# techmum21p/hybrid-rag-ColBERTv2

Hardware: AMD Instinct MI355X
Metric: queries/sec + p50 retrieval latency, 1M-chunk corpus, top-10 rerank (higher is better)
Workload: dtype fp32 (faithful: bf16 hi/lo split, fp32 accumulate)

## Files before the change

hybrid-rag-colbertv2_amd/_lib.py:

```python
from __future__ import annotations

import ctypes
import os
import re

PKG = os.path.dirname(os.path.abspath(__file__))
LIB_PATH = os.path.join(PKG, "libcolbert_mi355x.so")
HEADER = os.path.join(os.path.dirname(PKG), "include", "colbert_mi355x.h")

DTYPE_BF16 = 1
DTYPE_F32 = 2
DTYPE_MXFP8 = 3
SCORER_MAXSIM = 0
SCORER_REF_MEANPOOL_COSINE = 1
SCORERS = {"maxsim": SCORER_MAXSIM, "ref_meanpool_cosine": SCORER_REF_MEANPOOL_COSINE}
ERR_EINVAL, ERR_EUNSUPPORTED, ERR_EHIP, ERR_ESTATE = -1, -2, -3, -4
F32_SCORE, F32_SEARCH, F32_RERANK = 0, 1, 2
(OPT_FUSED_TOPK, OPT_DYNAMIC_TAIL, OPT_BAND_DOC_MAJOR, OPT_BAND_LOWER_BOUND, OPT_TOPK_BMAX, OPT_BAND_FUSED,
 OPT_RESCORE_SPLIT, OPT_BAND_REUSE, OPT_BAND_BLOCK_SKIP, OPT_RESCORE_GRID, OPT_DENSE_DOCS, OPT_P1_COLLECT_FUSED,
 OPT_FOLD_KEYS, OPT_FILTER_PATH, OPT_FILTER_BATCH_CHUNK_DOCS, OPT_FILTER_BAND) = (1, 2, 3, 4, 5, 6, 7, 8, 9, 10, 11, 12,
                                                                                 13, 14, 15, 16)
FILTER_AUTO, FILTER_SUBSET, FILTER_DENSE = 0, 1, 2
FILTER_BAND_AUTO, FILTER_BAND_ON, FILTER_BAND_OFF = 0, 1, 2

_p, _i32, _i64, _sz = ctypes.c_void_p, ctypes.c_int32, ctypes.c_int64, ctypes.c_size_t
_SIGS = {
    "cbv2_abi_version": (ctypes.c_int, []),
    "cbv2_last_error": (ctypes.c_char_p, []),
    "cbv2_build_stamp": (ctypes.c_char_p, []),
    "cbv2_index_create": (ctypes.c_int, [ctypes.c_int, _p, _i32, _i64, _i32, _i32, _p, _i64,
                                         ctypes.POINTER(ctypes.c_void_p)]),
    "cbv2_index_destroy": (ctypes.c_int, [_p]),
    "cbv2_hbm_alloc": (ctypes.c_int, [ctypes.c_int, ctypes.c_size_t, ctypes.POINTER(ctypes.c_void_p),
                                      ctypes.POINTER(ctypes.c_int32)]),
    "cbv2_hbm_free": (ctypes.c_int, [ctypes.c_int, _p]),
    "cbv2_index_time_scans": (ctypes.c_int, [_p, _i32]),
# ... 139 lines not shown
```

hybrid-rag-colbertv2_amd/csrc/colbert_mi355x.hip:

```cpp
#include <hip/hip_runtime.h>

#include <stdarg.h>
#include <stdint.h>

#include <algorithm>
#include <atomic>
#include <mutex>
#include <type_traits>
#include <vector>
#include <stdio.h>
#include <string.h>

#include "colbert_mi355x.h"

namespace {

constexpr int kDim = 128;
constexpr int kLd = 128;
constexpr int kLqMax = 32;
constexpr int kRowBytes = kDim * 2;
constexpr int kDocBytes = kLd * kRowBytes;
constexpr int kTopkMax = 1024;
constexpr int kSmallMax = 1024;
constexpr int kMergeMax = 8192;
// ... 3516 lines not shown
  }
  __syncthreads();
  if (wave == 0) {
    const float m0 = fmaxf(fmaxf(s_m[0][c16], s_m[1][c16]), fmaxf(s_m[2][c16], s_m[3][c16]));
    const float m1 = fmaxf(fmaxf(s_m[0][16 + c16], s_m[1][16 + c16]), fmaxf(s_m[2][16 + c16], s_m[3][16 + c16]));
    const float v = dpp_row_sum16((c16 < lq ? m0 : 0.0f) + (16 + c16 < lq ? m1 : 0.0f));
    if (lane == 0) {
      raw[(size_t)b * C + c] = v;
      if (raw_words.w != nullptr) raw_words.put((size_t)b * C + c, (int32_t)__float_as_uint(v), 0.0f);
    }
  }
}

constexpr float kBoundUp = 1.0f + 1.0f / 1024.0f;
constexpr float kAccSlack = 1.0f / 4096.0f;

__device__ __forceinline__ void split_row8(const float* __restrict__ src, uint16_t* __restrict__ hi,
                                           uint16_t* __restrict__ lo, int sub, float& xx, float& rr, float& hh) {
  const f32x4* s4 = reinterpret_cast<const f32x4*>(src + 8 * sub);
  const f32x4 v0 = s4[0], v1 = s4[1];
  float x[8] = {v0[0], v0[1], v0[2], v0[3], v1[0], v1[1], v1[2], v1[3]};
  uint16_t h[8], l[8];
  xx = rr = hh = 0.0f;
#pragma unroll
  for (int e = 0; e < 8; ++e) {
    const __bf16 bh = (__bf16)x[e];
    const float fh = (float)bh;
    const float r = x[e] - fh;
    const __bf16 bl = (__bf16)r;
    h[e] = __builtin_bit_cast(uint16_t, bh);
// ... 45 lines not shown
}

constexpr int kArriveSlotsK = 4;
constexpr int kArrPhase1K = 3;
constexpr int64_t kSplitZeroInts = 16384;
__global__ __launch_bounds__(512) void split_query_kernel(const float* __restrict__ Q, int lq,
                                                          uint16_t* __restrict__ qhi, uint16_t* __restrict__ qlo,
                                                          float E, float M, float* __restrict__ beta,
                                                          int32_t* __restrict__ count = nullptr,
                                                          uint32_t* __restrict__ lbu = nullptr,
                                                          int32_t* __restrict__ done = nullptr, int count0 = 0,
                                                          int32_t* __restrict__ arrive = nullptr, int narrive = 0,
                                                          int* __restrict__ ctr = nullptr, int nctr = 0,
                                                          uint32_t ready_seq = 0, int nrows = 0,
                                                          uint32_t* __restrict__ zkeys = nullptr, int64_t nz = 0,
                                                          int32_t* __restrict__ ready_words = nullptr) {
  __shared__ float s_t[kLqMax];
  const int b = blockIdx.x, tid = threadIdx.x, r = tid >> 4, sub = tid & 15;
  if (nrows > 0 && b >= nrows) {
    const int64_t per = kSplitZeroInts, i0 = (int64_t)(b - nrows) * per;
    for (int64_t i = i0 + 4 * tid; i < i0 + per && i < nz; i += 4 * blockDim.x) {
      if (i + 3 < nz)
        *reinterpret_cast<uint4*>(zkeys + i) = make_uint4(0u, 0u, 0u, 0u);
      else
        for (int64_t e = i; e < nz; ++e) zkeys[e] = 0u;
    }
    return;
  }
  if (r < lq) {
    const size_t row = (size_t)b * lq + r;
    float xx, rr, hh;
    split_row8(Q + row * kDim, qhi + row * kDim, qlo + row * kDim, sub, xx, rr, hh);
    const float nq = sqrtf(xx) * kBoundUp, eq = sqrtf(rr) * kBoundUp;
    const float t = nq * E + eq * M + kAccSlack * (nq + eq) * M;
    if (sub == 0) s_t[r] = t;
  }
  __syncthreads();
  if (tid == 0) {
    float a[4];
#pragma unroll
    for (int g = 0; g < 4; ++g) {
      a[g] = 0.0f;
      for (int rr = g; rr < lq; rr += 4) a[g] += s_t[rr];
    }
    beta[b] = ((a[0] + a[1]) + (a[2] + a[3])) * kBoundUp;
    if (count != nullptr) count[b] = count0;
    if (lbu != nullptr) lbu[b] = 0xffffffffu;
    if (done != nullptr) done[b] = 0;
  }
  if (arrive != nullptr) {
    const int per = narrive / kArriveSlotsK;
    for (int i = tid; i < narrive; i += blockDim.x) {
      const int j = i / per, e = i - j * per;
      arrive[((size_t)j * nrows + b) * per + e] = 0;
    }
  }
  if (ctr != nullptr && b == 0)
    for (int i = tid; i < nctr; i += blockDim.x) ctr[i] = 0;
  if (ready_seq != 0 && ready_words != nullptr) {
    __syncthreads();
// ... 125 lines not shown
      if (16 * rt < dlb) {
        const f32x4 init = (dlb >= 16 * rt + 16) ? f32x4{} : row_mask_init16(16 * rt + 4 * g, dlb);
        tile16_x3(ah[t], al[t], qh, ql, init, m);
      }
    }
  }
  const float w0 = fold16_max(fold32_max(m[0])), w1 = fold16_max(fold32_max(m[1]));
  if (lane < 16) {
    s_m[wave][lane] = w0;
    s_m[wave][16 + lane] = w1;
  }
  __syncthreads();
  float v = 0.0f;
  if (wave == 0) {
    float m0 = s_m[0][c16], m1 = s_m[0][16 + c16];
#pragma unroll
    for (int w = 1; w < NW; ++w) {
      m0 = fmaxf(m0, s_m[w][c16]);
      m1 = fmaxf(m1, s_m[w][16 + c16]);
    }
    v = dpp_row_sum16((c16 < lq ? m0 : 0.0f) + (16 + c16 < lq ? m1 : 0.0f));
  }
  __syncthreads();
  return v;
}

struct RowSelect {
  int mode = 0;
  int32_t* arrive = nullptr;
  int k = 0;
// ... 83 lines not shown
    int r = 0;
    for (int j = 0; j < m; ++j) r += sel[j] > key ? 1 : 0;
    if (r < k) {
      os[r] = u2f((uint32_t)(key >> 32));
      oi[r] = (int32_t)(id_base + (int64_t)(~(uint32_t)key));
      if (mirror.w != nullptr) mirror.put(r, oi[r], os[r]);
    }
  }
  for (int j = m + tid; j < k; j += nth) {
    os[j] = neg_inf();
    oi[j] = -1;
    if (mirror.w != nullptr) mirror.put(j, -1, neg_inf());
  }
}

template <bool LONG = false, int NW = 4>
__global__ __launch_bounds__(NW * 64, 2) void rescore_split_kernel(
    const uint8_t* __restrict__ hi, const uint8_t* __restrict__ lo, const int32_t* __restrict__ doclens, int64_t n,
    int64_t id_base, const uint16_t* __restrict__ qhi, const uint16_t* __restrict__ qlo, int lq,
    const int32_t* __restrict__ cand, const int32_t* __restrict__ count, int64_t limit, int64_t ld_c,
    float* __restrict__ out, int64_t ld_out, const int32_t* __restrict__ only_neg, int ld,
    uint32_t* __restrict__ lb_min, int64_t c0, float* __restrict__ fb_T = nullptr, int32_t* __restrict__ fb_done = nullptr,
    int fb_k = 0, float* __restrict__ fb_s = nullptr, int32_t* __restrict__ fb_i = nullptr, RowSelect rs = RowSelect(),
    TaggedCand tc = TaggedCand()) {
  __shared__ float s_m[4][32];
  __shared__ uint64_t sel[kTopkMax];
  __shared__ uint32_t hist[2048];
  __shared__ uint32_t s_bin, s_above, s_bincount, s_cnt;
  __shared__ uint32_t misc[8];
  __shared__ int s_last;
  __shared__ int32_t s_cid;
  const int lane = threadIdx.x & 63;
  const int wave = __builtin_amdgcn_readfirstlane(threadIdx.x >> 6);
  const int b = blockIdx.y;
  if (rs.stamps != nullptr && threadIdx.x == 0 && blockIdx.x < kLabWgs)
    rs.stamps[16 + 2 * blockIdx.x] = __builtin_amdgcn_s_memrealtime();
  if (only_neg != nullptr && only_neg[b] >= 0) return;
  int64_t lim = limit;
  if (count != nullptr) {
// ... 16 lines not shown
      __threadfence();
      const int kk = (int)((int64_t)fb_k < n ? fb_k : n);
      topk_exact_row(row, n, kk, sel, hist, &s_bin, &s_above, &s_bincount, &s_cnt);
      sort_and_write(sel, kk, fb_k, id_base, fb_s + (size_t)b * fb_k, fb_i + (size_t)b * fb_k,
                     rs.ids_mirror.row(b, fb_k));
      if (rs.mode == kSelBand && threadIdx.x == 0) rs.status[b] = cb >= kWaitTimedOut ? -2 : -1;
      return;
    }
  }
  const bool idle = c0 + (int64_t)blockIdx.x >= lim;
  if (idle && rs.mode == kSelNone) return;
  if (!idle) {
    bf16x8 qh[2][4], ql[2][4];
    load_qfrag16(qhi, b, b + 1, lq, lane, qh);
    load_qfrag16(qlo, b, b + 1, lq, lane, ql);
    for (int64_t c = c0 + blockIdx.x; c < lim; c += gridDim.x) {
      int64_t id;
      if (tc.w != nullptr) {
        if (threadIdx.x == 0) {
          s_cid = wait_tagged(tc.w + (size_t)b * ld_c + c, tc);
          if (rs.mode != kSelNone)
            st_sc1(reinterpret_cast<uint32_t*>(const_cast<int32_t*>(cand)) + (size_t)b * ld_c + c, (uint32_t)s_cid);
        }
        __syncthreads();
        id = s_cid;
        __syncthreads();
      } else {
        id = cand ? (int64_t)cand[b * ld_c + c] : id_base + c;
      }
      const int64_t loc = id - id_base;
      float v = neg_inf();
      if (id >= 0 && loc >= 0 && loc < n)
        v = faithful_doc_split<LONG, NW>(hi, lo, loc, ld, doclens[loc], qh, ql, lane, wave, lq, s_m);
      if (threadIdx.x == 0) {
        if (rs.mode != kSelNone)
          st_sc1(out + (size_t)b * ld_out + c, v);
        else
          out[(size_t)b * ld_out + c] = v;
        if (rs.raw.w != nullptr) rs.raw.put((size_t)b * ld_c + c, (int32_t)__float_as_uint(v), 0.0f);
        if (lb_min != nullptr) atomicMin(lb_min + b, f2u(v));
      }
    }
  }
  if (rs.stamps != nullptr && threadIdx.x == 0 && blockIdx.x < kLabWgs)
    rs.stamps[17 + 2 * blockIdx.x] = __builtin_amdgcn_s_memrealtime();
  if (rs.mode == kSelNone) return;
  if (!row_last_arrival(rs.arrive + (size_t)b * kArriveInts, (int)gridDim.x, 8, &s_last)) return;
  lab_stamp(rs.stamps, 6);
// ... 331 lines not shown
      __syncthreads();
    }
    d = d_next;
  }
}

__device__ __forceinline__ float band_threshold(int b, const float* __restrict__ lb, const uint32_t* __restrict__ lbu,
                                                const float* __restrict__ topk_s, int k,
                                                const float* __restrict__ beta) {
  if (lbu != nullptr) return u2f(lbu[b]) - beta[b];
  if (lb != nullptr) return lb[b] - beta[b];
  return topk_s[(size_t)b * k + k - 1] - 2.0f * beta[b];
}

constexpr int kBandLds = 2048;
__global__ __launch_bounds__(256) void band_collect_kernel(const float* __restrict__ T, int64_t n,
                                                           const float* __restrict__ topk_s, int k,
                                                           const float* __restrict__ beta, int64_t id_base,
                                                           int cap, int32_t* __restrict__ cand,
                                                           int32_t* __restrict__ count,
                                                           const float* __restrict__ lb,
                                                           const uint32_t* __restrict__ lbu,
                                                           const int32_t* __restrict__ topk_i,
                                                           const uint32_t* __restrict__ bm,
                                                           uint64_t* __restrict__ stamps = nullptr) {
  __shared__ int32_t s_ids[kBandLds];
  __shared__ int s_n, s_base;
  const int b = blockIdx.y, lane = threadIdx.x & 63;
  if (stamps != nullptr && threadIdx.x == 0 && blockIdx.x < kLabWgs)
    stamps[16 + 2 * blockIdx.x] = __builtin_amdgcn_s_memrealtime();
  if (threadIdx.x == 0) s_n = 0;
  __syncthreads();
  const float thr = band_threshold(b, lb, lbu, topk_s, k, beta);
  const float* row = T + (size_t)b * n;
  int32_t* crow = cand + (size_t)b * cap;
  uint64_t kth = 0;
  if (topk_i != nullptr) {
    kth = rank_key(topk_s[(size_t)b * k + k - 1], (uint32_t)((int64_t)topk_i[(size_t)b * k + k - 1] - id_base));
    if (blockIdx.x == 0)
      for (int j = threadIdx.x; j < k; j += blockDim.x) crow[j] = topk_i[(size_t)b * k + j];
  }
  auto offer = [&](int64_t i, float v) {
    const bool take = i < n && v >= thr && (topk_i == nullptr || rank_key(v, (uint32_t)i) < kth);
    const uint64_t mask = __ballot(take);
    if (mask == 0) return;
    const int nh = __popcll(mask);
    int base = 0;
    if (lane == 0) base = atomicAdd(&s_n, nh);
    base = __shfl(base, 0);
    const int pos = base + __popcll(mask & ((1ull << lane) - 1ull));
    if (take) {
      if (pos < kBandLds) {
        s_ids[pos] = (int32_t)(id_base + i);
      } else {
        const int gp = atomicAdd(count + b, 1);
        if (gp < cap) crow[gp] = (int32_t)(id_base + i);
      }
    }
  };
  if (bm != nullptr) {
    const int64_t nb = (n + 63) >> 6;
    const uint32_t* krow = bm + (size_t)b * nb;
    const uint32_t uthr = f2u(thr);
    const int wave = threadIdx.x >> 6, nw = blockDim.x >> 6;
    const int c16 = lane & 15, r4 = lane >> 4;
    const bool vec = (n & 3) == 0 && (reinterpret_cast<uintptr_t>(T) & 15) == 0;
    for (int64_t g0 = (int64_t)blockIdx.x * 64; g0 < nb; g0 += (int64_t)gridDim.x * 64) {
      const int64_t kb = g0 + lane;
      const uint64_t qual = __ballot(kb < nb && krow[kb] >= uthr);
      uint64_t mine = 0;
      int q = 0;
      for (uint64_t m = qual; m != 0; m &= m - 1, ++q)
        if (q % nw == wave) mine |= m & (~m + 1);
      while (mine != 0) {
        int64_t i0[4];
#pragma unroll
        for (int s4 = 0; s4 < 4; ++s4) {
          int64_t blk = -1;
#pragma unroll
          for (int u = 0; u < 4; ++u) {
            const int64_t bu = mine != 0 ? g0 + (__ffsll((long long)mine) - 1) : -1;
            if (mine != 0) mine &= mine - 1;
            if (u == r4) blk = bu;
          }
          i0[s4] = blk >= 0 ? (blk << 6) + 4 * c16 : n;
        }
        float v[4][4];
#pragma unroll
        for (int s4 = 0; s4 < 4; ++s4) {
          if (vec && i0[s4] + 3 < n) {
            const f32x4 x4 = *reinterpret_cast<const f32x4*>(row + i0[s4]);
            v[s4][0] = x4[0], v[s4][1] = x4[1], v[s4][2] = x4[2], v[s4][3] = x4[3];
          } else {
#pragma unroll
            for (int e = 0; e < 4; ++e) v[s4][e] = i0[s4] + e < n ? row[i0[s4] + e] : 0.0f;
          }
        }
#pragma unroll
        for (int s4 = 0; s4 < 4; ++s4)
#pragma unroll
          for (int e = 0; e < 4; ++e) offer(i0[s4] + e < n ? i0[s4] + e : n, v[s4][e]);
      }
    }
  } else {
    constexpr int U = 8;
    const int64_t step = (int64_t)gridDim.x * blockDim.x * U;
    for (int64_t i0 = (int64_t)blockIdx.x * blockDim.x * U; i0 < n; i0 += step) {
      float v[U];
#pragma unroll
      for (int u = 0; u < U; ++u) {
        const int64_t i = i0 + (int64_t)u * blockDim.x + threadIdx.x;
        v[u] = i < n ? row[i] : 0.0f;
      }
#pragma unroll
      for (int u = 0; u < U; ++u) offer(i0 + (int64_t)u * blockDim.x + threadIdx.x, v[u]);
    }
  }
// ... 466 lines not shown
  int* task_ring = nullptr;
  uint32_t task_seq = 0;
  hipEvent_t ring_ev[128] = {};
  bool ring_ev_used[128] = {};
  int64_t last_plan[4] = {0, 0, 0, 0};
  bool fused_topk = false;
  int fused_topk_mode = 0;
  int dynamic_tail = 1;
  int topk_bmax = 1;
  int band_doc_major = 0;
  bool band_lower_bound = true;
  bool band_fused = false;
  bool rescore_split = true;
  bool band_reuse = true;
  bool band_block_skip = true;
  int rescore_grid = 0;
  bool dense_docs = false;
  bool p1_collect_fused = true;
  bool fold_keys = true;
  std::mutex mu;
  const uint8_t* resid = nullptr;
  float resid_max = 0.0f, norm_max = 0.0f;
  bool time_scans = false;
  uint64_t* clk = nullptr;
  bool clock_on = false;
  size_t scan_ev_used = 0;
  std::vector<hipEvent_t> scan_ev;
  size_t band_ev_used = 0;
  bool band_open = false;
  std::vector<hipEvent_t> band_ev;
// ... 865 lines not shown
  int32_t* done = nullptr;
  int32_t* arrive = nullptr;
  int32_t* cand = nullptr;
  float* F = nullptr;
  void* tk = nullptr;
  size_t tk_bytes = 0;
  float* T = nullptr;
  int32_t* dcnt = nullptr;
  int32_t* doff = nullptr;
  int32_t* act = nullptr;
  int32_t* act_off = nullptr;
  int32_t* act_cnt = nullptr;
  int32_t* dctr = nullptr;
  int32_t* pair_b = nullptr;
  int32_t* pair_c = nullptr;
};

constexpr int kArriveSlots = kArriveSlotsK;
constexpr int kArrBmax = 0, kArrBand = 1, kArrRerank = 2, kArrPhase1 = kArrPhase1K;
inline int32_t* arrive_row0(const F32Ws& w, int slot, int B) { return w.arrive + (size_t)slot * B * kArriveInts; }

size_t f32_ws_layout(const cbv2_index* ix, int op, int B, int lq, int cap, uint8_t* base, F32Ws* w) {
  size_t off = 0;
  auto take = [&](size_t bytes) -> uint8_t* {
    uint8_t* p = base ? base + off : nullptr;
    off += (bytes + 255) & ~(size_t)255;
    return p;
  };
  const size_t qbytes = (size_t)B * lq * kDim * sizeof(uint16_t);
  if (op == CBV2_F32_SEARCH) w->ctr = (int*)take(kCtrBytes);
// ... 8 lines not shown
    w->done = (int32_t*)take((size_t)B * sizeof(int32_t));
    w->cand = (int32_t*)take((size_t)B * cap * sizeof(int32_t));
    w->F = (float*)take((size_t)B * cap * sizeof(float));
    w->tk_bytes = std::max(topk_ws_bytes(B, ix->n), bm_ws_bytes(B, ix->n));
    w->tk = take(w->tk_bytes);
    w->T = (float*)take((size_t)B * (size_t)(ix->n > 0 ? ix->n : 1) * sizeof(float));
    const size_t nd = (size_t)(ix->n > 0 ? ix->n : 1) * sizeof(int32_t);
    w->dcnt = (int32_t*)take(nd);
    w->doff = (int32_t*)take(nd);
    w->act = (int32_t*)take(nd);
    w->act_off = (int32_t*)take(nd);
    w->act_cnt = (int32_t*)take(nd);
    w->dctr = (int32_t*)take(2 * sizeof(int32_t));
    w->pair_b = (int32_t*)take((size_t)B * cap * sizeof(int32_t));
    w->pair_c = (int32_t*)take((size_t)B * cap * sizeof(int32_t));
  }
  return off;
}

int check_f32(cbv2_index* ix, int op, const float* Q, int32_t B, int32_t lq, int32_t cap, void* ws, size_t wsb,
              F32Ws* w) {
  CBV2_REQUIRE(ix != nullptr, "null index");
  if (ix->resid == nullptr) return fail(CBV2_ESTATE, "index has no fp32 residual (cbv2_index_attach_residual)");
  CBV2_REQUIRE(Q != nullptr && aligned16(Q), "query pointer must be non-null and 16-byte aligned");
  CBV2_REQUIRE(B >= 1 && B <= 65535, "B must be in [1, 65535] (got %d)", B);
  CBV2_REQUIRE(lq >= 1 && lq <= kLqMax, "lq must be in [1, %d] (got %d)", kLqMax, lq);
  const size_t need = f32_ws_layout(ix, op, B, lq, cap, nullptr, w);
  CBV2_REQUIRE(ws != nullptr && wsb >= need && aligned16(ws), "workspace too small or misaligned (%zu < %zu)",
               wsb, need);
  f32_ws_layout(ix, op, B, lq, cap, (uint8_t*)ws, w);
// ... 30 lines not shown
}

int split_queries(cbv2_index* ix, const float* Q, int B, int lq, F32Ws* w, hipStream_t st, int count0 = 0,
                  bool zero_ctr = false, uint32_t* zkeys = nullptr, int64_t nz = 0) {
  note_split(ix, Q, B, lq, w->qhi);
  const int64_t extra = zkeys != nullptr ? (nz + kSplitZeroInts - 1) / kSplitZeroInts : 0;
  const bool publish = g_split_ready_seq != 0 && g_split_ready_word != nullptr;
  if (publish) {
    g_ready_flag = g_split_ready_word;
    g_ready_flag_ld = 1;
  }
  hipLaunchKernelGGL(split_query_kernel, dim3((unsigned)(B + extra)), dim3(512), 0, st, Q, lq, w->qhi, w->qlo,
                     ix->resid_max, ix->norm_max, w->beta, w->count, reinterpret_cast<uint32_t*>(w->lb), w->done,
                     count0, w->arrive, kArriveSlots * kArriveInts, zero_ctr ? w->ctr : nullptr,
                     zero_ctr ? kRingInts : 0, publish ? g_split_ready_seq : 0u, B, zkeys, nz,
                     publish ? g_split_ready_word : nullptr);
  return launch_check("split_query_kernel");
}

constexpr int64_t kRsSmallPairs = 4096;
constexpr int64_t kRsSplitGrid = 1024;
struct RescoreGrid { unsigned gx; bool two; };
RescoreGrid rescore_grid(const cbv2_index* ix, int B, int64_t span) {
  const int64_t grid_auto = std::min<int64_t>(kRsSplitGrid, std::max<int64_t>(256, 4096 / std::max(B, 1)));
  const int64_t grid_max = ix->rescore_grid > 0 ? ix->rescore_grid : grid_auto;
  const unsigned gx = (unsigned)(span < grid_max ? span : grid_max);
  return {gx, ix->ld == kLd && (int64_t)gx * B > 3LL * cu_count(ix->device)};
}
int launch_rescore(cbv2_index* ix, const F32Ws* w, int B, int lq, const int32_t* cand, const int32_t* count,
                   int64_t limit, int64_t ld_c, float* out, int64_t ld_out, hipStream_t st,
                   const int32_t* only_neg = nullptr, int pw = 0, uint32_t* lb_min = nullptr, int64_t c0 = 0,
                   float* fb_T = nullptr, int32_t* fb_done = nullptr, int fb_k = 0, float* fb_s = nullptr,
                   int32_t* fb_i = nullptr, const RowSelect& rs = RowSelect(), TaggedCand tc = TaggedCand()) {
  if (limit <= c0 && fb_T == nullptr && rs.mode == kSelNone) return CBV2_OK;
  if (ix->rescore_split) {
    int64_t span = limit - c0;
    if (fb_T != nullptr) span = std::max<int64_t>(span, std::min<int64_t>(ix->n, 256));
    if (span < 1) span = 1;
    const auto [gx, two] = rescore_grid(ix, B, span);
    auto kern = ix->ld != kLd ? rescore_split_kernel<true, 4>
                              : (two ? rescore_split_kernel<false, 2> : rescore_split_kernel<false, 4>);
    hipLaunchKernelGGL(kern, dim3(gx, (unsigned)B), dim3(two ? 128 : 256), 0, st, ix->tokens, ix->resid, ix->doclens,
                       ix->n, ix->id_base, w->qhi, w->qlo, lq, cand, count, limit, ld_c, out, ld_out, only_neg,
                       (int)ix->ld, lb_min, c0, fb_T, fb_done, fb_k, fb_s, fb_i, rs, tc);
    return launch_check("rescore_split_kernel");
  }
  if (c0 != 0 || fb_T != nullptr || rs.mode != kSelNone || tc.w != nullptr)
    return fail(CBV2_EUNSUPPORTED, "pair offset / fallback / row select need the split rescoring");
  if (pw <= 0) pw = (int64_t)B * limit <= kRsSmallPairs ? 1 : kRsPerWave;
  const int64_t per_wg = 4LL * pw;
  int64_t gx = (limit + per_wg - 1) / per_wg;
  gx = gx < 1024 ? gx : 1024;
  hipLaunchKernelGGL(ix->ld != kLd ? rescore_x3_kernel<true> : rescore_x3_kernel<false>, dim3((unsigned)gx, (unsigned)B),
                     dim3(256), 0, st, ix->tokens, ix->resid,
                     ix->doclens, ix->n, ix->id_base, w->qhi, w->qlo, lq, cand, count, limit, ld_c, out, ld_out,
                     only_neg, (int)ix->ld, pw, lb_min);
  return launch_check("rescore_x3_kernel");
}

// ... 246 lines not shown
      if (B <= 16) return launch_f8x4_ids<nt(kF8W4Q4), 3>(ix, f, Qb, Qs, B, lq, out, st);
      return launch_f8x4_ids<kF8W4Q4, 3>(ix, f, Qb, Qs, B, lq, out, st);
    case kF8ShapeW4Q8: return launch_f8x4_ids<kF8W4Q8, 2>(ix, f, Qb, Qs, B, lq, out, st);
    default: return launch_f8x4_ids<with_d(kF8W8Q8, 1), 1>(ix, f, Qb, Qs, B, lq, out, st);
  }
}

int rescore_subset(cbv2_index* ix, const cbv2_filter* f, const F32Ws* w, int B, int lq, float* out, hipStream_t st,
                   const int32_t* only_neg = nullptr) {
  const int64_t span = only_neg != nullptr ? std::min<int64_t>(f->m, std::max<int64_t>(64, 256 / B)) : f->m;
  const auto [gx, two] = rescore_grid(ix, B, span);
  auto kern = two ? rescore_split_kernel<false, 2> : rescore_split_kernel<false, 4>;
  hipLaunchKernelGGL(kern, dim3(gx, (unsigned)B), dim3(two ? 128 : 256), 0, st, ix->tokens, ix->resid, ix->doclens,
                     ix->n, (int64_t)0, w->qhi, w->qlo, lq, f->ids, (const int32_t*)nullptr, f->m, (int64_t)0, out,
                     f->m, only_neg, (int)ix->ld, (uint32_t*)nullptr, (int64_t)0, (float*)nullptr,
                     (int32_t*)nullptr, 0, (float*)nullptr, (int32_t*)nullptr, RowSelect(), TaggedCand());
  return launch_check("rescore_split_kernel (subset)");
}

constexpr double kFilterSubsetMaxFrac = 0.5;
constexpr double kFilterSubsetMaxFracF8 = 0.5;
bool filter_takes_subset(const cbv2_index* ix, int64_t m_allowed, int32_t scorer) {
  const bool f8 = ix->dtype == CBV2_DTYPE_MXFP8;
  const bool supported = scorer == CBV2_SCORER_MAXSIM && (ix->dtype == CBV2_DTYPE_BF16 || f8) && ix->ld == kLd;
  const double frac = f8 ? kFilterSubsetMaxFracF8 : kFilterSubsetMaxFrac;
  return supported &&
         (ix->filter_path == 1 || (ix->filter_path == 0 && (double)m_allowed <= frac * (double)ix->n));
}

constexpr int64_t kFilterBandMinSavedPairs = 4000;
constexpr int64_t kFilterBandSavedPairsPerK = 16;
// ... 195 lines not shown
  const int64_t grid = (fb->chunks + C.waves - 1) / C.waves;
  if (grid < 1 || grid > 0x0fffffff) return fail(CBV2_EUNSUPPORTED, "scan grid too large");
  hipLaunchKernelGGL(maxsim_scan_f8_stream_kernel<C>, dim3((unsigned)grid), dim3(C.waves * 64), 0, st, ix->tokens,
                     ix->scales, ix->doclens, (int64_t)0, Qb, Qb + (size_t)B * lq * kDim, B, lq, out, M,
                     fb->chunk_docs, (int)ix->ld, (const int32_t*)nullptr, fb->table);
  return launch_check("maxsim_scan_f8_stream_kernel (ragged)");
}

int rescore_ragged(cbv2_index* ix, const cbv2_filter_batch* fb, const F32Ws* w, int B, int lq, const int32_t* cand,
                   float* out, int64_t M, hipStream_t st) {
  const auto [gx, two] = rescore_grid(ix, B, M);
  auto kern = two ? rescore_split_kernel<false, 2> : rescore_split_kernel<false, 4>;
  hipLaunchKernelGGL(kern, dim3(gx, (unsigned)B), dim3(two ? 128 : 256), 0, st, ix->tokens, ix->resid, ix->doclens,
                     ix->n, (int64_t)0, w->qhi, w->qlo, lq, cand, fb->table + fb_off_count(B), M, M, out, M,
                     (const int32_t*)nullptr, (int)ix->ld, (uint32_t*)nullptr, (int64_t)0, (float*)nullptr,
                     (int32_t*)nullptr, 0, (float*)nullptr, (int32_t*)nullptr, RowSelect(), TaggedCand());
  return launch_check("rescore_split_kernel (ragged)");
}

FilterPlan filter_batch_plan(const cbv2_index* ix, const cbv2_filter_batch* fb, int32_t B, int32_t lq,
                             int32_t scorer) {
  return filter_plan_m(ix, fb->max_m, true, B, lq, scorer);
}
}

extern "C" {

int cbv2_set_error(int code, const char* msg) { return fail(code, "%s", msg); }

int cbv2_abi_version(void) { return CBV2_ABI_VERSION; }

// ... 577 lines not shown
      return CBV2_OK;
    case CBV2_OPT_TOPK_BMAX:
      ix->topk_bmax = (int)value;
      return CBV2_OK;
    case CBV2_OPT_BAND_FUSED:
      ix->band_fused = value != 0;
      return CBV2_OK;
    case CBV2_OPT_RESCORE_SPLIT:
      ix->rescore_split = value != 0;
      return CBV2_OK;
    case CBV2_OPT_BAND_REUSE:
      ix->band_reuse = value != 0;
      return CBV2_OK;
    case CBV2_OPT_BAND_BLOCK_SKIP:
      ix->band_block_skip = value != 0;
      return CBV2_OK;
    case CBV2_OPT_DENSE_DOCS:
      ix->dense_docs = value != 0;
      return CBV2_OK;
    case CBV2_OPT_P1_COLLECT_FUSED:
      ix->p1_collect_fused = value != 0;
      return CBV2_OK;
    case CBV2_OPT_FOLD_KEYS:
      ix->fold_keys = value != 0;
      return CBV2_OK;
    case CBV2_OPT_FILTER_PATH:
      if (value < 0 || value > 2) return fail(CBV2_EINVAL, "filter path must be 0 (automatic), 1 (subset) or 2 (dense)");
      ix->filter_path = (int)value;
      return CBV2_OK;
    case CBV2_OPT_FILTER_BAND:
// ... 328 lines not shown
  } else {
    RowSelect rs;
    if (fb_fused && B <= kBandPairMaxB) {
      rs.mode = kSelBand;
      rs.arrive = arrive_row0(w, kArrBand, B);
      rs.k = k;
      rs.out_s = out_scores;
      rs.out_i = out_ids;
      rs.lb = lb;
      rs.lbu = lbu;
      rs.status = out_status;
      rs.ids_mirror = g_ids_mirror;
      if (g_ids_mirror.w != nullptr) g_ids_mirror_used = true;
      rs.stamps = LAB_STAMPS(3);
    }
    if ((rc = launch_rescore(ix, &w, B, lq, w.cand, w.count, cap, cap, w.F, cap, st, nullptr,
                             B <= kBandPairMaxB ? 1 : 0, nullptr, c0, fb_fused ? w.T : nullptr,
                             fb_fused ? w.done : nullptr, k, out_scores, out_ids, rs)))
      return rc;
    if (rs.mode != kSelNone) return CBV2_OK;
  }
  hipLaunchKernelGGL(band_select_kernel, dim3((unsigned)B), dim3(kTkThreads), 0, st, w.F, w.cand, w.count, cap, k,
                     ix->id_base, out_scores, out_ids, out_status, lb, lbu);
  if ((rc = launch_check("band_select_kernel"))) return rc;
  if (fb_fused) return CBV2_OK;
  if (ix->rescore_split && k <= kTopkMax) {
    const int64_t fb = std::max<int64_t>(64, 256 / B);
    const unsigned gx = (unsigned)(ix->n < fb ? ix->n : fb);
    hipLaunchKernelGGL(ix->ld != kLd ? fallback_split_kernel<true> : fallback_split_kernel<false>, dim3(gx, (unsigned)B),
                       dim3(256), 0, st, ix->tokens, ix->resid, ix->doclens, ix->n, ix->id_base, w.qhi, w.qlo, lq,
                       w.T, out_status, (int)ix->ld, w.done, k, out_scores, out_ids);
    return launch_check("fallback_split_kernel");
  }
// ... 293 lines not shown
```

hybrid-rag-colbertv2_amd/index.py:

```python
from __future__ import annotations

import ctypes
import json
import os
from typing import Iterable, List, Optional, Sequence, Tuple, Union

import torch

from . import _lib

LD = 128
LONG_LDS = (128, 256, 512, 1024)
DIM = 128
LQ_MAX = 32
BAND_CAP = 16384


_raw_stream = getattr(torch._C, "_cuda_getCurrentRawStream", None)


def _stream_ptr(device: torch.device) -> int:
    if _raw_stream is not None:
        return _raw_stream(device.index if device.index is not None else torch.cuda.current_device())
    return torch.cuda.current_stream(device).cuda_stream
# ... 297 lines not shown
        _require_cuda(doclens, "doclens")
        if doclens.dtype != torch.int32 or doclens.shape != (x.shape[0],):
            raise ValueError("doclens must be int32 [n]")
        doclens = doclens.contiguous()
        _lib.check(_lib.lib().cbv2_split_f32(x.data_ptr(), x.numel() // DIM, x.shape[1], doclens.data_ptr(),
                                             hi.data_ptr(), lo.data_ptr(), bounds.data_ptr(), _stream_ptr(x.device)))
        b = bounds.tolist()
        return cls(hi, doclens, id_base=id_base, residual=lo, bounds=(b[0], b[1]))

    def _f32_ws(self, op: int, B: int, lq: int, cap: int) -> torch.Tensor:
        need = int(_lib.lib().cbv2_f32_workspace_bytes(self._h, op, B, lq, cap))
        if self._ws is None or self._ws.numel() * 4 < need:
            self._ws = torch.empty(((need + 3) // 4,), dtype=torch.float32, device=self.device)
        return self._ws

    @classmethod
    def mxfp8(cls, tokens: torch.Tensor, doclens: torch.Tensor, id_base: int = 0) -> "ColbertIndex":
        q, sc = quantize_mxfp8(tokens)
        return cls(q, doclens, id_base=id_base, scales=sc)

    @classmethod
    def from_embeddings(cls, embs, device="cuda", id_base: int = 0, build_means: bool = False,
                        dtype: str = "bf16"):
        device = torch.device(device)
        if dtype not in ("bf16", "fp8", "fp32"):
            raise ValueError(f"index dtype must be bf16, fp8 or fp32 (got {dtype!r})")
        tokens, doclens = pack_tokens(embs, device, ld=None,
                                      dtype=torch.float32 if dtype == "fp32" else torch.bfloat16)
        if dtype == "fp32":
            ix = cls.faithful_f32(tokens, doclens, id_base=id_base)
# ... 311 lines not shown
        _lib.check(L.cbv2_search(self._h, sid, qptr, qdt, B, lq, int(k), self._ws.data_ptr(),
                                 self._ws.numel() * 4, out_s.data_ptr(), out_i.data_ptr(),
                                 _stream_ptr(self.device)))
        return out_s, out_i

    def _search_f32(self, Qd: torch.Tensor, B: int, lq: int, k: int, cap: int = BAND_CAP):
        cap = max(int(cap), int(k))
        ws = self._f32_ws(_lib.F32_SEARCH, B, lq, cap)
        out_s = torch.empty((B, k), dtype=torch.float32, device=self.device)
        out_i = torch.empty((B, k), dtype=torch.int32, device=self.device)
        status = torch.empty((B,), dtype=torch.int32, device=self.device)
        _lib.check(_lib.lib().cbv2_search_f32(self._h, Qd.data_ptr(), B, lq, int(k), cap, ws.data_ptr(),
                                              ws.numel() * 4, out_s.data_ptr(), out_i.data_ptr(),
                                              status.data_ptr(), _stream_ptr(self.device)))
        self.last_band = status
        return out_s, out_i

    def _search_f32_global(self, Qd: torch.Tensor, B: int, lq: int, k: int, lb_reduce, cap: int = BAND_CAP):
        cap = max(int(cap), int(k))
        ws = self._f32_ws(_lib.F32_SEARCH, B, lq, cap)
        out_s = torch.empty((B, k), dtype=torch.float32, device=self.device)
        out_i = torch.empty((B, k), dtype=torch.int32, device=self.device)
        status = torch.empty((B,), dtype=torch.int32, device=self.device)
        fk = torch.empty((B, k), dtype=torch.float32, device=self.device)
        L = _lib.lib()
        _lib.check(L.cbv2_search_f32_begin(self._h, Qd.data_ptr(), B, lq, int(k), cap, ws.data_ptr(),
                                           ws.numel() * 4, fk.data_ptr(), out_s.data_ptr(), out_i.data_ptr(),
                                           status.data_ptr(), _stream_ptr(self.device)))
        lb = lb_reduce(fk).to(device=self.device, dtype=torch.float32).contiguous()
        if tuple(lb.shape) != (B,):
            raise ValueError(f"lb_reduce must return f32 [{B}] (got {tuple(lb.shape)})")
        _lib.check(L.cbv2_search_f32_finish(self._h, B, lq, int(k), cap, ws.data_ptr(), ws.numel() * 4,
                                            lb.data_ptr(), out_s.data_ptr(), out_i.data_ptr(), status.data_ptr(),
                                            _stream_ptr(self.device)))
        self.last_band = status
        return out_s, out_i

    def rerank(self, Q: torch.Tensor, cand: torch.Tensor, k: int):
        blocks = self._query_blocks(Q, "maxsim")
        if blocks is not None:
            raw = self.rerank(blocks[0], cand, 0).clone()
            for q in blocks[1:]:
                raw += self.rerank(q, cand, 0)
            if k == 0:
                return raw
            cand = cand.to(device=self.device, dtype=torch.int32)
            return select_topk(raw, int(k), ids=cand if cand.dim() == 2 else cand.unsqueeze(0))
        _keep, qptr, _, Bq, lq = self._prep_query(Q, "maxsim")
        cand = cand.to(device=self.device, dtype=torch.int32).contiguous()
        if cand.dim() == 1:
# ... 233 lines not shown
```

include/colbert_mi355x.h:

```cpp
#ifndef COLBERT_MI355X_H
#define COLBERT_MI355X_H

#include <stddef.h>
#include <stdint.h>

#ifdef __cplusplus
extern "C" {
#endif

#define CBV2_ABI_VERSION 2

#define CBV2_DTYPE_BF16 1
#define CBV2_DTYPE_F32 2
#define CBV2_DTYPE_MXFP8 3

#define CBV2_SCORER_MAXSIM 0
#define CBV2_SCORER_REF_MEANPOOL_COSINE 1

#define CBV2_OK 0
#define CBV2_EINVAL -1
#define CBV2_EUNSUPPORTED -2
#define CBV2_EHIP -3
#define CBV2_ESTATE -4

// ... 19 lines not shown
#define CBV2_OPT_DYNAMIC_TAIL 2
#define CBV2_OPT_BAND_DOC_MAJOR 3
#define CBV2_OPT_BAND_LOWER_BOUND 4
#define CBV2_OPT_TOPK_BMAX 5
#define CBV2_OPT_BAND_FUSED 6
#define CBV2_OPT_RESCORE_SPLIT 7
#define CBV2_OPT_BAND_REUSE 8
#define CBV2_OPT_BAND_BLOCK_SKIP 9
#define CBV2_OPT_RESCORE_GRID 10
#define CBV2_OPT_DENSE_DOCS 11
#define CBV2_OPT_P1_COLLECT_FUSED 12
#define CBV2_OPT_FOLD_KEYS 13
#define CBV2_OPT_FILTER_PATH 14
#define CBV2_OPT_FILTER_BATCH_CHUNK_DOCS 15
#define CBV2_OPT_FILTER_BAND 16
int cbv2_index_set_option(cbv2_index* index, int32_t option, int64_t value);
int cbv2_index_last_scan_plan(const cbv2_index* index, int64_t* out4);
int64_t cbv2_search_fused_slots(const cbv2_index* index, int32_t B, int32_t k, int32_t scorer);

int cbv2_index_create_mxfp8(int device, const void* tokens, const void* scales, int64_t n, int32_t ld,
                            int32_t d, const int32_t* doclens, int64_t id_base, cbv2_index** out);

int cbv2_quantize_mxfp8(const void* x, int32_t dtype, int64_t rows, void* q, void* scales, void* stream);

int cbv2_index_build_means(cbv2_index* index, const float* tokens_f32, int32_t ld_src,
                           float* doc_means, void* stream);

int cbv2_score(cbv2_index* index, int32_t scorer, const void* Q, int32_t q_dtype, int32_t B,
               int32_t lq, float* out, int64_t ld_out, void* stream);

// ... 184 lines not shown
```

Before: 1747.

## Add hi-first bound certification to band rescore and compact band-collect block scan

In the band rescore, each candidate doc is first scored with only the bf16 hi tokens against both query halves. A precomputed per-query error bound (beta_a) then rules out docs whose upper bound cannot reach the current lower bound, so the lo fragments are loaded and the full three-product MFMA runs only for docs that survive. Separately, band_collect now gives each block a contiguous key range, compacts qualifying 64-doc blocks into an LDS list via ballot and atomics, and spreads them across waves. The cost is an extra partial MFMA pass for docs that are not skipped, extra syncthreads, extra workspace, and reliance on the correctness of the bound.

```diff
diff --git a/hybrid-rag-colbertv2_amd/_lib.py b/hybrid-rag-colbertv2_amd/_lib.py
--- a/hybrid-rag-colbertv2_amd/_lib.py
+++ b/hybrid-rag-colbertv2_amd/_lib.py
@@ -20,6 +20,7 @@
  OPT_RESCORE_SPLIT, OPT_BAND_REUSE, OPT_BAND_BLOCK_SKIP, OPT_RESCORE_GRID, OPT_DENSE_DOCS, OPT_P1_COLLECT_FUSED,
  OPT_FOLD_KEYS, OPT_FILTER_PATH, OPT_FILTER_BATCH_CHUNK_DOCS, OPT_FILTER_BAND) = (1, 2, 3, 4, 5, 6, 7, 8, 9, 10, 11, 12,
                                                                                  13, 14, 15, 16)
+OPT_BAND_HI_FIRST = 17
 FILTER_AUTO, FILTER_SUBSET, FILTER_DENSE = 0, 1, 2
 FILTER_BAND_AUTO, FILTER_BAND_ON, FILTER_BAND_OFF = 0, 1, 2
 
diff --git a/hybrid-rag-colbertv2_amd/csrc/colbert_mi355x.hip b/hybrid-rag-colbertv2_amd/csrc/colbert_mi355x.hip
--- a/hybrid-rag-colbertv2_amd/csrc/colbert_mi355x.hip
+++ b/hybrid-rag-colbertv2_amd/csrc/colbert_mi355x.hip
@@ -3554,6 +3554,7 @@
 
 constexpr float kBoundUp = 1.0f + 1.0f / 1024.0f;
 constexpr float kAccSlack = 1.0f / 4096.0f;
+constexpr float kRoundUpBf16 = 1.0f + 1.0f / 256.0f;
 
 __device__ __forceinline__ void split_row8(const float* __restrict__ src, uint16_t* __restrict__ hi,
                                            uint16_t* __restrict__ lo, int sub, float& xx, float& rr, float& hh) {
@@ -3629,7 +3630,10 @@
                                                           int* __restrict__ ctr = nullptr, int nctr = 0,
                                                           uint32_t ready_seq = 0, int nrows = 0,
                                                           uint32_t* __restrict__ zkeys = nullptr, int64_t nz = 0,
-                                                          int32_t* __restrict__ ready_words = nullptr) {
+                                                          int32_t* __restrict__ ready_words = nullptr,
+                                                          float* __restrict__ beta_a = nullptr,
+                                                          int32_t* __restrict__ skipped = nullptr) {
+  __shared__ float s_a[kLqMax];
   __shared__ float s_t[kLqMax];
   const int b = blockIdx.x, tid = threadIdx.x, r = tid >> 4, sub = tid & 15;
   if (nrows > 0 && b >= nrows) {
@@ -3648,7 +3652,11 @@
     split_row8(Q + row * kDim, qhi + row * kDim, qlo + row * kDim, sub, xx, rr, hh);
     const float nq = sqrtf(xx) * kBoundUp, eq = sqrtf(rr) * kBoundUp;
     const float t = nq * E + eq * M + kAccSlack * (nq + eq) * M;
-    if (sub == 0) s_t[r] = t;
+    if (sub == 0) {
+      s_t[r] = t;
+      const float nh = sqrtf(hh) * kBoundUp, nl = eq * kRoundUpBf16;
+      s_a[r] = nh * (E * kRoundUpBf16) + kAccSlack * (nh + nl) * M;
+    }
   }
   __syncthreads();
   if (tid == 0) {
@@ -3659,6 +3667,12 @@
       for (int rr = g; rr < lq; rr += 4) a[g] += s_t[rr];
     }
     beta[b] = ((a[0] + a[1]) + (a[2] + a[3])) * kBoundUp;
+    if (beta_a != nullptr) {
+      float s = 0.0f;
+      for (int rr = 0; rr < lq; ++rr) s += s_a[rr];
+      beta_a[b] = s * kBoundUp;
+    }
+    if (skipped != nullptr) skipped[b] = 0;
     if (count != nullptr) count[b] = count0;
     if (lbu != nullptr) lbu[b] = 0xffffffffu;
     if (done != nullptr) done[b] = 0;
@@ -3814,6 +3828,92 @@
   float v = 0.0f;
   if (wave == 0) {
     float m0 = s_m[0][c16], m1 = s_m[0][16 + c16];
+#pragma unroll
+    for (int w = 1; w < NW; ++w) {
+      m0 = fmaxf(m0, s_m[w][c16]);
+      m1 = fmaxf(m1, s_m[w][16 + c16]);
+    }
+    v = dpp_row_sum16((c16 < lq ? m0 : 0.0f) + (16 + c16 < lq ? m1 : 0.0f));
+  }
+  __syncthreads();
+  return v;
+}
+
+struct HiFirst {
+  const uint32_t* lbu = nullptr;
+  const float* lb = nullptr;
+  const float* beta_a = nullptr;
+  int32_t* skipped = nullptr;
+};
+
+template <int NW>
+__device__ __forceinline__ float faithful_doc_split_hi_first(const uint8_t* __restrict__ hi,
+                                                             const uint8_t* __restrict__ lo, int64_t loc, int dl,
+                                                             const bf16x8 (&qh)[2][4], const bf16x8 (&ql)[2][4],
+                                                             int lane, int wave, int lq, float (&s_m)[4][32],
+                                                             float lbv, float beta_a, bool& ruled_out) {
+  constexpr int TPW = 8 / NW;
+  const int g = lane >> 4, c16 = lane & 15;
+  const size_t at = (size_t)loc * kLd * kRowBytes;
+  bf16x8 ah[TPW][4], al[TPW][4];
+#pragma unroll
+  for (int t = 0; t < TPW; ++t) gbl_afrag16(hi + at, TPW * wave + t, lane, ah[t]);
+  dl = dl < 0 ? 0 : (dl > kLd ? kLd : dl);
+  float m[2] = {neg_inf(), neg_inf()};
+#pragma unroll
+  for (int t = 0; t < TPW; ++t) {
+    const int rt = TPW * wave + t;
+    if (16 * rt < dl) {
+      const f32x4 init = (dl >= 16 * rt + 16) ? f32x4{} : row_mask_init16(16 * rt + 4 * g, dl);
+#pragma unroll
+      for (int ct = 0; ct < 2; ++ct) {
+        f32x4 acc = init;
+#pragma unroll
+        for (int s = 0; s < 4; ++s) acc = __builtin_amdgcn_mfma_f32_16x16x32_bf16(ah[t][s], ql[ct][s], acc, 0, 0, 0);
+#pragma unroll
+        for (int s = 0; s < 4; ++s) acc = __builtin_amdgcn_mfma_f32_16x16x32_bf16(ah[t][s], qh[ct][s], acc, 0, 0, 0);
+        m[ct] = fmaxf(fmaxf(m[ct], fmaxf(acc[0], acc[1])), fmaxf(acc[2], acc[3]));
+      }
+    }
+  }
+  float w0 = fold16_max(fold32_max(m[0])), w1 = fold16_max(fold32_max(m[1]));
+  if (lane < 16) {
+    s_m[wave][lane] = w0;
+    s_m[wave][16 + lane] = w1;
+  }
+  __syncthreads();
+  float m0 = s_m[0][c16], m1 = s_m[0][16 + c16];
+#pragma unroll
+  for (int w = 1; w < NW; ++w) {
+    m0 = fmaxf(m0, s_m[w][c16]);
+    m1 = fmaxf(m1, s_m[w][16 + c16]);
+  }
+  const float sa = dpp_row_sum16((c16 < lq ? m0 : 0.0f) + (16 + c16 < lq ? m1 : 0.0f));
+  ruled_out = __builtin_amdgcn_readfirstlane((int)(sa + beta_a < lbv)) != 0;
+  __syncthreads();
+  if (ruled_out) return neg_inf();
+#pragma unroll
+  for (int t = 0; t < TPW; ++t) gbl_afrag16(lo + at, TPW * wave + t, lane, al[t]);
+  m[0] = m[1] = neg_inf();
+#pragma unroll
+  for (int t = 0; t < TPW; ++t) {
+    const int rt = TPW * wave + t;
+    if (16 * rt < dl) {
+      const f32x4 init = (dl >= 16 * rt + 16) ? f32x4{} : row_mask_init16(16 * rt + 4 * g, dl);
+      tile16_x3(ah[t], al[t], qh, ql, init, m);
+    }
+  }
+  w0 = fold16_max(fold32_max(m[0]));
+  w1 = fold16_max(fold32_max(m[1]));
+  if (lane < 16) {
+    s_m[wave][lane] = w0;
+    s_m[wave][16 + lane] = w1;
+  }
+  __syncthreads();
+  float v = 0.0f;
+  if (wave == 0) {
+    m0 = s_m[0][c16];
+    m1 = s_m[0][16 + c16];
 #pragma unroll
     for (int w = 1; w < NW; ++w) {
       m0 = fmaxf(m0, s_m[w][c16]);
@@ -3927,7 +4027,7 @@
   }
 }
 
-template <bool LONG = false, int NW = 4>
+template <bool LONG = false, int NW = 4, bool HF = false>
 __global__ __launch_bounds__(NW * 64, 2) void rescore_split_kernel(
     const uint8_t* __restrict__ hi, const uint8_t* __restrict__ lo, const int32_t* __restrict__ doclens, int64_t n,
     int64_t id_base, const uint16_t* __restrict__ qhi, const uint16_t* __restrict__ qlo, int lq,
@@ -3935,7 +4035,8 @@
     float* __restrict__ out, int64_t ld_out, const int32_t* __restrict__ only_neg, int ld,
     uint32_t* __restrict__ lb_min, int64_t c0, float* __restrict__ fb_T = nullptr, int32_t* __restrict__ fb_done = nullptr,
     int fb_k = 0, float* __restrict__ fb_s = nullptr, int32_t* __restrict__ fb_i = nullptr, RowSelect rs = RowSelect(),
-    TaggedCand tc = TaggedCand()) {
+    TaggedCand tc = TaggedCand(), HiFirst hf = HiFirst()) {
+  static_assert(!(HF && LONG), "hi-first certification: 128-slot docs only");
   __shared__ float s_m[4][32];
   __shared__ uint64_t sel[kTopkMax];
   __shared__ uint32_t hist[2048];
@@ -3982,6 +4083,11 @@
     bf16x8 qh[2][4], ql[2][4];
     load_qfrag16(qhi, b, b + 1, lq, lane, qh);
     load_qfrag16(qlo, b, b + 1, lq, lane, ql);
+    float hf_lb = 0.0f, hf_beta = 0.0f;
+    if constexpr (HF) {
+      hf_lb = hf.lbu != nullptr ? u2f(hf.lbu[b]) : hf.lb[b];
+      hf_beta = hf.beta_a[b];
+    }
     for (int64_t c = c0 + blockIdx.x; c < lim; c += gridDim.x) {
       int64_t id;
       if (tc.w != nullptr) {
@@ -3998,8 +4104,16 @@
       }
       const int64_t loc = id - id_base;
       float v = neg_inf();
-      if (id >= 0 && loc >= 0 && loc < n)
-        v = faithful_doc_split<LONG, NW>(hi, lo, loc, ld, doclens[loc], qh, ql, lane, wave, lq, s_m);
+      if constexpr (HF) {
+        bool ruled_out = false;
+        if (id >= 0 && loc >= 0 && loc < n)
+          v = faithful_doc_split_hi_first<NW>(hi, lo, loc, doclens[loc], qh, ql, lane, wave, lq, s_m, hf_lb, hf_beta,
+                                              ruled_out);
+        if (ruled_out && threadIdx.x == 0) atomicAdd(hf.skipped + b, 1);
+      } else {
+        if (id >= 0 && loc >= 0 && loc < n)
+          v = faithful_doc_split<LONG, NW>(hi, lo, loc, ld, doclens[loc], qh, ql, lane, wave, lq, s_m);
+      }
       if (threadIdx.x == 0) {
         if (rs.mode != kSelNone)
           st_sc1(out + (size_t)b * ld_out + c, v);
@@ -4361,6 +4475,8 @@
 }
 
 constexpr int kBandLds = 2048;
+constexpr int kBandKeyU = 8;
+constexpr int kBandKeys = 256 * kBandKeyU;
 __global__ __launch_bounds__(256) void band_collect_kernel(const float* __restrict__ T, int64_t n,
                                                            const float* __restrict__ topk_s, int k,
                                                            const float* __restrict__ beta, int64_t id_base,
@@ -4372,11 +4488,12 @@
                                                            const uint32_t* __restrict__ bm,
                                                            uint64_t* __restrict__ stamps = nullptr) {
   __shared__ int32_t s_ids[kBandLds];
-  __shared__ int s_n, s_base;
+  __shared__ int32_t s_blk[kBandKeys];
+  __shared__ int s_n, s_base, s_nb;
   const int b = blockIdx.y, lane = threadIdx.x & 63;
   if (stamps != nullptr && threadIdx.x == 0 && blockIdx.x < kLabWgs)
     stamps[16 + 2 * blockIdx.x] = __builtin_amdgcn_s_memrealtime();
-  if (threadIdx.x == 0) s_n = 0;
+  if (threadIdx.x == 0) s_n = s_nb = 0;
   __syncthreads();
   const float thr = band_threshold(b, lb, lbu, topk_s, k, beta);
   const float* row = T + (size_t)b * n;
@@ -4405,6 +4522,7 @@
       }
     }
   };
+  static_assert(kBandKeys == 256 * kBandKeyU, "band_collect_kernel runs 256 threads");
   if (bm != nullptr) {
     const int64_t nb = (n + 63) >> 6;
     const uint32_t* krow = bm + (size_t)b * nb;
@@ -4412,24 +4530,35 @@
     const int wave = threadIdx.x >> 6, nw = blockDim.x >> 6;
     const int c16 = lane & 15, r4 = lane >> 4;
     const bool vec = (n & 3) == 0 && (reinterpret_cast<uintptr_t>(T) & 15) == 0;
-    for (int64_t g0 = (int64_t)blockIdx.x * 64; g0 < nb; g0 += (int64_t)gridDim.x * 64) {
-      const int64_t kb = g0 + lane;
-      const uint64_t qual = __ballot(kb < nb && krow[kb] >= uthr);
-      uint64_t mine = 0;
-      int q = 0;
-      for (uint64_t m = qual; m != 0; m &= m - 1, ++q)
-        if (q % nw == wave) mine |= m & (~m + 1);
-      while (mine != 0) {
+    const int64_t per = (nb + gridDim.x - 1) / gridDim.x;
+    const int64_t s0 = (int64_t)blockIdx.x * per;
+    const int64_t s1 = s0 + per < nb ? s0 + per : nb;
+    for (int64_t k0 = s0; k0 < s1; k0 += kBandKeys) {
+      uint32_t kv[kBandKeyU];
+#pragma unroll
+      for (int u = 0; u < kBandKeyU; ++u) {
+        const int64_t kb = k0 + u * (kBandKeys / kBandKeyU) + threadIdx.x;
+        kv[u] = kb < s1 ? krow[kb] : 0u;
+      }
+#pragma unroll
+      for (int u = 0; u < kBandKeyU; ++u) {
+        const int64_t kb = k0 + u * (kBandKeys / kBandKeyU) + threadIdx.x;
+        const bool qual = kb < s1 && kv[u] >= uthr;
+        const uint64_t mask = __ballot(qual);
+        if (mask == 0) continue;
+        int base = 0;
+        if (lane == 0) base = atomicAdd(&s_nb, __popcll(mask));
+        base = __shfl(base, 0);
+        if (qual) s_blk[base + __popcll(mask & ((1ull << lane) - 1ull))] = (int32_t)kb;
+      }
+      __syncthreads();
+      const int nq = s_nb;
+      for (int q0 = 16 * wave; q0 < nq; q0 += 16 * nw) {
         int64_t i0[4];
 #pragma unroll
         for (int s4 = 0; s4 < 4; ++s4) {
-          int64_t blk = -1;
-#pragma unroll
-          for (int u = 0; u < 4; ++u) {
-            const int64_t bu = mine != 0 ? g0 + (__ffsll((long long)mine) - 1) : -1;
-            if (mine != 0) mine &= mine - 1;
-            if (u == r4) blk = bu;
-          }
+          const int q = q0 + 4 * s4 + r4;
+          const int64_t blk = q < nq ? (int64_t)s_blk[q] : -1;
           i0[s4] = blk >= 0 ? (blk << 6) + 4 * c16 : n;
         }
         float v[4][4];
@@ -4448,6 +4577,9 @@
 #pragma unroll
           for (int e = 0; e < 4; ++e) offer(i0[s4] + e < n ? i0[s4] + e : n, v[s4][e]);
       }
+      __syncthreads();
+      if (threadIdx.x == 0) s_nb = 0;
+      __syncthreads();
     }
   } else {
     constexpr int U = 8;
@@ -4944,6 +5076,7 @@
   bool rescore_split = true;
   bool band_reuse = true;
   bool band_block_skip = true;
+  bool band_hi_first = true;
   int rescore_grid = 0;
   bool dense_docs = false;
   bool p1_collect_fused = true;
@@ -5839,6 +5972,8 @@
   int32_t* dctr = nullptr;
   int32_t* pair_b = nullptr;
   int32_t* pair_c = nullptr;
+  float* beta_a = nullptr;
+  int32_t* skipped = nullptr;
 };
 
 constexpr int kArriveSlots = kArriveSlotsK;
@@ -5877,6 +6012,8 @@
     w->dctr = (int32_t*)take(2 * sizeof(int32_t));
     w->pair_b = (int32_t*)take((size_t)B * cap * sizeof(int32_t));
     w->pair_c = (int32_t*)take((size_t)B * cap * sizeof(int32_t));
+    w->beta_a = (float*)take((size_t)B * sizeof(float));
+    w->skipped = (int32_t*)take((size_t)B * sizeof(int32_t));
   }
   return off;
 }
@@ -5937,7 +6074,7 @@
                      ix->resid_max, ix->norm_max, w->beta, w->count, reinterpret_cast<uint32_t*>(w->lb), w->done,
                      count0, w->arrive, kArriveSlots * kArriveInts, zero_ctr ? w->ctr : nullptr,
                      zero_ctr ? kRingInts : 0, publish ? g_split_ready_seq : 0u, B, zkeys, nz,
-                     publish ? g_split_ready_word : nullptr);
+                     publish ? g_split_ready_word : nullptr, w->beta_a, w->skipped);
   return launch_check("split_query_kernel");
 }
 
@@ -5954,18 +6091,21 @@
                    int64_t limit, int64_t ld_c, float* out, int64_t ld_out, hipStream_t st,
                    const int32_t* only_neg = nullptr, int pw = 0, uint32_t* lb_min = nullptr, int64_t c0 = 0,
                    float* fb_T = nullptr, int32_t* fb_done = nullptr, int fb_k = 0, float* fb_s = nullptr,
-                   int32_t* fb_i = nullptr, const RowSelect& rs = RowSelect(), TaggedCand tc = TaggedCand()) {
+                   int32_t* fb_i = nullptr, const RowSelect& rs = RowSelect(), TaggedCand tc = TaggedCand(),
+                   const HiFirst& hf = HiFirst()) {
   if (limit <= c0 && fb_T == nullptr && rs.mode == kSelNone) return CBV2_OK;
   if (ix->rescore_split) {
     int64_t span = limit - c0;
     if (fb_T != nullptr) span = std::max<int64_t>(span, std::min<int64_t>(ix->n, 256));
     if (span < 1) span = 1;
     const auto [gx, two] = rescore_grid(ix, B, span);
+    const bool hi_first = hf.beta_a != nullptr && ix->ld == kLd;
     auto kern = ix->ld != kLd ? rescore_split_kernel<true, 4>
+                : hi_first    ? (two ? rescore_split_kernel<false, 2, true> : rescore_split_kernel<false, 4, true>)
                               : (two ? rescore_split_kernel<false, 2> : rescore_split_kernel<false, 4>);
     hipLaunchKernelGGL(kern, dim3(gx, (unsigned)B), dim3(two ? 128 : 256), 0, st, ix->tokens, ix->resid, ix->doclens,
                        ix->n, ix->id_base, w->qhi, w->qlo, lq, cand, count, limit, ld_c, out, ld_out, only_neg,
-                       (int)ix->ld, lb_min, c0, fb_T, fb_done, fb_k, fb_s, fb_i, rs, tc);
+                       (int)ix->ld, lb_min, c0, fb_T, fb_done, fb_k, fb_s, fb_i, rs, tc, hi_first ? hf : HiFirst());
     return launch_check("rescore_split_kernel");
   }
   if (c0 != 0 || fb_T != nullptr || rs.mode != kSelNone || tc.w != nullptr)
@@ -6242,7 +6382,7 @@
   hipLaunchKernelGGL(kern, dim3(gx, (unsigned)B), dim3(two ? 128 : 256), 0, st, ix->tokens, ix->resid, ix->doclens,
                      ix->n, (int64_t)0, w->qhi, w->qlo, lq, f->ids, (const int32_t*)nullptr, f->m, (int64_t)0, out,
                      f->m, only_neg, (int)ix->ld, (uint32_t*)nullptr, (int64_t)0, (float*)nullptr,
-                     (int32_t*)nullptr, 0, (float*)nullptr, (int32_t*)nullptr, RowSelect(), TaggedCand());
+                     (int32_t*)nullptr, 0, (float*)nullptr, (int32_t*)nullptr, RowSelect(), TaggedCand(), HiFirst());
   return launch_check("rescore_split_kernel (subset)");
 }
 
@@ -6468,7 +6608,7 @@
   hipLaunchKernelGGL(kern, dim3(gx, (unsigned)B), dim3(two ? 128 : 256), 0, st, ix->tokens, ix->resid, ix->doclens,
                      ix->n, (int64_t)0, w->qhi, w->qlo, lq, cand, fb->table + fb_off_count(B), M, M, out, M,
                      (const int32_t*)nullptr, (int)ix->ld, (uint32_t*)nullptr, (int64_t)0, (float*)nullptr,
-                     (int32_t*)nullptr, 0, (float*)nullptr, (int32_t*)nullptr, RowSelect(), TaggedCand());
+                     (int32_t*)nullptr, 0, (float*)nullptr, (int32_t*)nullptr, RowSelect(), TaggedCand(), HiFirst());
   return launch_check("rescore_split_kernel (ragged)");
 }
 
@@ -7076,6 +7216,9 @@
       return CBV2_OK;
     case CBV2_OPT_BAND_BLOCK_SKIP:
       ix->band_block_skip = value != 0;
+      return CBV2_OK;
+    case CBV2_OPT_BAND_HI_FIRST:
+      ix->band_hi_first = value != 0;
       return CBV2_OK;
     case CBV2_OPT_DENSE_DOCS:
       ix->dense_docs = value != 0;
@@ -7434,9 +7577,17 @@
       if (g_ids_mirror.w != nullptr) g_ids_mirror_used = true;
       rs.stamps = LAB_STAMPS(3);
     }
+    HiFirst hf;
+    if (ix->band_hi_first && B > kBandPairMaxB && ix->ld == kLd && (lb != nullptr || lbu != nullptr) &&
+        w.beta_a != nullptr) {
+      hf.lb = lb;
+      hf.lbu = lbu;
+      hf.beta_a = w.beta_a;
+      hf.skipped = w.skipped;
+    }
     if ((rc = launch_rescore(ix, &w, B, lq, w.cand, w.count, cap, cap, w.F, cap, st, nullptr,
                              B <= kBandPairMaxB ? 1 : 0, nullptr, c0, fb_fused ? w.T : nullptr,
-                             fb_fused ? w.done : nullptr, k, out_scores, out_ids, rs)))
+                             fb_fused ? w.done : nullptr, k, out_scores, out_ids, rs, TaggedCand(), hf)))
       return rc;
     if (rs.mode != kSelNone) return CBV2_OK;
   }
diff --git a/hybrid-rag-colbertv2_amd/index.py b/hybrid-rag-colbertv2_amd/index.py
--- a/hybrid-rag-colbertv2_amd/index.py
+++ b/hybrid-rag-colbertv2_amd/index.py
@@ -335,6 +335,18 @@
             self._ws = torch.empty(((need + 3) // 4,), dtype=torch.float32, device=self.device)
         return self._ws
 
+    def _note_band_skipped(self, ws: torch.Tensor, B: int, lq: int, cap: int) -> None:
+        need = int(_lib.lib().cbv2_f32_workspace_bytes(self._h, _lib.F32_SEARCH, B, lq, cap))
+        off = (need - ((4 * B + 255) & ~255)) // 4
+        self._band_skipped = (ws, off, B)
+
+    @property
+    def last_band_skipped(self) -> Optional[torch.Tensor]:
+        if getattr(self, "_band_skipped", None) is None:
+            return None
+        ws, off, B = self._band_skipped
+        return ws[off:off + B].view(torch.int32).clone()
+
     @classmethod
     def mxfp8(cls, tokens: torch.Tensor, doclens: torch.Tensor, id_base: int = 0) -> "ColbertIndex":
         q, sc = quantize_mxfp8(tokens)
@@ -676,6 +688,7 @@
                                               ws.numel() * 4, out_s.data_ptr(), out_i.data_ptr(),
                                               status.data_ptr(), _stream_ptr(self.device)))
         self.last_band = status
+        self._note_band_skipped(ws, B, lq, cap)
         return out_s, out_i
 
     def _search_f32_global(self, Qd: torch.Tensor, B: int, lq: int, k: int, lb_reduce, cap: int = BAND_CAP):
@@ -696,6 +709,7 @@
                                             lb.data_ptr(), out_s.data_ptr(), out_i.data_ptr(), status.data_ptr(),
                                             _stream_ptr(self.device)))
         self.last_band = status
+        self._note_band_skipped(ws, B, lq, cap)
         return out_s, out_i
 
     def rerank(self, Q: torch.Tensor, cand: torch.Tensor, k: int):
diff --git a/include/colbert_mi355x.h b/include/colbert_mi355x.h
--- a/include/colbert_mi355x.h
+++ b/include/colbert_mi355x.h
@@ -57,6 +57,7 @@
 #define CBV2_OPT_FILTER_PATH 14
 #define CBV2_OPT_FILTER_BATCH_CHUNK_DOCS 15
 #define CBV2_OPT_FILTER_BAND 16
+#define CBV2_OPT_BAND_HI_FIRST 17
 int cbv2_index_set_option(cbv2_index* index, int32_t option, int64_t value);
 int cbv2_index_last_scan_plan(const cbv2_index* index, int64_t* out4);
 int64_t cbv2_search_fused_slots(const cbv2_index* index, int32_t B, int32_t k, int32_t scorer);
```

After: 1746. Within noise of the previous version (-0.1%).
